# pavlidic/Binary-SpGEMM

Hardware: AMD Instinct MI355X
Metric: output nnz/sec (GNZ/s) (higher is better)
Workload: dtype int32; 1 GPU; R-MAT scale 22, edge factor 16, (a,b,c,d)=(0.30,0.25,0.25,0.20), seed 1, A*A; n=4194304, nnz_a=67108664, products=1336443900, nnz_c=1336366087, parallelism=row-shards x1 cut at equal work, B replicated, priming_steps=0, flow=auto, full=False

## Files before the change

### binary-spgemm_amd/csrc/context.hip

```cpp
#include "internal.hpp"

using namespace bsp;

thread_local char bspgemm_err_text[512] = "";

extern "C" const char *bspgemm_last_error(void) { return g_err; }

extern "C" const char *bspgemm_status_string(bspgemm_status s)
{
    switch (s) {
    case BSPGEMM_OK: return "ok";
    case BSPGEMM_ERR_INVALID: return "invalid argument";
    case BSPGEMM_ERR_ALLOC: return "allocation failed";
    case BSPGEMM_ERR_HIP: return "HIP runtime error";
    case BSPGEMM_ERR_NO_DEVICE: return "no gfx950 device (this library has no CPU fallback)";
    case BSPGEMM_ERR_OVERFLOW: return "result exceeds the int32 drop-in interface";
    case BSPGEMM_ERR_IO: return "file I/O error";
    case BSPGEMM_ERR_FORMAT: return "Matrix Market banner rejected";
    case BSPGEMM_ERR_SIZE: return "Matrix Market size line or entry rejected";
    case BSPGEMM_ERR_COMM: return "RCCL error";
    }
    return "unknown status";
}

// ... 25 lines not shown
        drop();
        hipFree(m->d_col_pad); hipFree(m->d_row_ptr_pad); hipFree(m->d_ext);
        m->d_col_pad = nullptr; m->d_row_ptr_pad = nullptr; m->d_ext = nullptr;
        return st;
    };
    HIPCHK_B(hipMalloc(reinterpret_cast<void **>(&plen), rows * sizeof(int)));
    HIPCHK_B(hipMalloc(reinterpret_cast<void **>(&pp64), (rows + 1) * sizeof(long long)));
    HIPCHK_B(hipMalloc(reinterpret_cast<void **>(&partials), (rows / 2048 + 4) * sizeof(long long)));
    launch_pad_lengths(m->d_row_ptr, m->rows, plen, s);
    launch_scan_counts(plen, m->rows, pp64, partials, nullptr, s);
    long long total = 0;
    HIPCHK_B(hipMemcpyAsync(&total, pp64 + rows, sizeof(long long), hipMemcpyDeviceToHost, s));
    HIPCHK_B(hipStreamSynchronize(s));
    if (total > 0x7fffffffll - 64 || (force < 0 && total > 2 * m->nnz)) { drop(); return BSPGEMM_OK; }
    hipError_t e = hipMalloc(reinterpret_cast<void **>(&m->d_col_pad), ((size_t)total + 64) * sizeof(int));
    if (e == hipSuccess) e = hipMalloc(reinterpret_cast<void **>(&m->d_row_ptr_pad), (rows + 1) * sizeof(int));
    if (e == hipSuccess) e = hipMalloc(reinterpret_cast<void **>(&m->d_ext), rows * sizeof(int2));
    if (e != hipSuccess) {
        (void)hipGetLastError();
        if (force == 1) { snprintf(g_err, sizeof g_err, "padded copy of col_idx: %s", hipGetErrorString(e)); return bail(BSPGEMM_ERR_ALLOC); }
        (void)bail(BSPGEMM_OK);
        return BSPGEMM_OK;
    }
    launch_narrow_row_ptr(pp64, m->d_row_ptr_pad, m->rows + 1, s);
    launch_pad_copy(m->d_row_ptr, m->d_col_idx, m->d_row_ptr_pad, m->rows, m->d_col_pad, m->d_ext, s);
    HIPCHK_B(hipGetLastError());
    HIPCHK_B(hipStreamSynchronize(s));
    drop();
    m->nnz_pad = total;
    m->pad_state = 1;
    return BSPGEMM_OK;
}

bspgemm_status ensure_blk8(const bspgemm_matrix *m)
{
    if (m->blk8_state) return BSPGEMM_OK;
    m->blk8_state = 2;
    const int force = m->ctx->rw_blk;
    if (force == 0 || (force < 0 && m->rows < (1 << 21))) return BSPGEMM_OK;
    const size_t ints = (size_t)3 * (((size_t)m->rows + 7) / 8 + 1);
    HIPCHK(hipMalloc(reinterpret_cast<void **>(&m->d_blk8), (ints + 4) * sizeof(int)));
    unsigned long long *d_clamped = reinterpret_cast<unsigned long long *>(m->d_blk8 + ((ints + 1) & ~(size_t)1));
    HIPCHK(hipMemsetAsync(d_clamped, 0, sizeof(unsigned long long), m->ctx->stream));
    launch_blk8(m->d_row_ptr, m->pad_state == 1 ? m->d_row_ptr_pad : nullptr, m->rows, m->d_blk8, d_clamped, m->ctx->stream);
    HIPCHK(hipGetLastError());
    unsigned long long clamped = 0;
    HIPCHK(hipMemcpyAsync(&clamped, d_clamped, sizeof(clamped), hipMemcpyDeviceToHost, m->ctx->stream));
    HIPCHK(hipStreamSynchronize(m->ctx->stream));
    if (force == 1 || clamped * 8ull <= (unsigned long long)m->nnz) m->blk8_state = 1;
    return BSPGEMM_OK;
}

bspgemm_status use_device(bspgemm_context *ctx)
{
    HIPCHK(hipSetDevice(ctx->device));
    return BSPGEMM_OK;
}

extern "C" int bspgemm_device_count(void)
{
    int ndev = 0;
    if (hipGetDeviceCount(&ndev) != hipSuccess) { (void)hipGetLastError(); return 0; }
    return ndev;
}

extern "C" bspgemm_status bspgemm_create(int device, bspgemm_context **out)
{
    if (!out) return FAIL(BSPGEMM_ERR_INVALID, "ctx is NULL");
    *out = nullptr;
    int ndev = 0;
    if (hipGetDeviceCount(&ndev) != hipSuccess || ndev <= 0)
        return FAIL(BSPGEMM_ERR_NO_DEVICE, "no HIP device visible");
    if (device < 0 || device >= ndev) return FAIL(BSPGEMM_ERR_INVALID, "device index out of range");
    hipDeviceProp_t prop;
    HIPCHK(hipGetDeviceProperties(&prop, device));
    if (strncmp(prop.gcnArchName, "gfx950", 6) != 0) {
        snprintf(g_err, sizeof g_err, "device %d is %s; libbspgemm carries gfx950 code only", device,
                 prop.gcnArchName);
        return BSPGEMM_ERR_NO_DEVICE;
    }
    bspgemm_context *ctx = new (std::nothrow) bspgemm_context();
    if (!ctx) return FAIL(BSPGEMM_ERR_ALLOC, "context");
// ... 105 lines not shown
    HIPCHK_B(hipMalloc(reinterpret_cast<void **>(&m->d_col_idx), ((size_t)nnz + 1) * sizeof(int)));
    HIPCHK_B(hipMemcpyAsync(m->d_row_ptr, row_ptr, ((size_t)rows + 1) * sizeof(int), hipMemcpyHostToDevice, ctx->stream));
    if (nnz > 0)
        HIPCHK_B(hipMemcpyAsync(m->d_col_idx, col_idx + base, (size_t)nnz * sizeof(int), hipMemcpyHostToDevice, ctx->stream));
    launch_rebase_i32(m->d_row_ptr, rows + 1, (int)base, ctx->stream);
    if (bspgemm_status st = ensure_deg8(m)) return bail(st);
    HIPCHK_B(hipStreamSynchronize(ctx->stream));
    *out = m;
    return BSPGEMM_OK;
}

extern "C" bspgemm_status bspgemm_matrix_wrap_device(bspgemm_context *ctx, int rows, int cols, int64_t nnz,
                                                     const int *d_row_ptr, const int *d_col_idx,
                                                     bspgemm_matrix **out)
{
    if (!ctx || !out || !d_row_ptr || rows < 0 || cols < 0 || nnz < 0) return FAIL(BSPGEMM_ERR_INVALID, "matrix_wrap_device");
    bspgemm_matrix *m = new (std::nothrow) bspgemm_matrix{ctx, rows, cols, (long long)nnz,
                                                          const_cast<int *>(d_row_ptr),
                                                          const_cast<int *>(d_col_idx), false};
    if (!m) return FAIL(BSPGEMM_ERR_ALLOC, "matrix");
    *out = m;
    return BSPGEMM_OK;
}

extern "C" void bspgemm_matrix_free(bspgemm_matrix *m)
{
    if (!m) return;
    hipSetDevice(m->ctx->device);
    if (m->owned) {
        hipFree(m->d_row_ptr);
        hipFree(m->d_col_idx);
    }
    hipFree(m->d_deg8);
    hipFree(m->d_blk8);
    hipFree(m->d_col_pad);
    hipFree(m->d_row_ptr_pad);
    hipFree(m->d_ext);
    delete m;
}
extern "C" bspgemm_status bspgemm_matrix_download(bspgemm_context *ctx, const bspgemm_matrix *m, int *row_ptr, int *col_idx)
{
    if (!ctx || !m || m->ctx != ctx) return FAIL(BSPGEMM_ERR_INVALID, "matrix_download");
    if (bspgemm_status st = use_device(ctx)) return st;
    if (row_ptr)
        HIPCHK(hipMemcpyAsync(row_ptr, m->d_row_ptr, ((size_t)m->rows + 1) * sizeof(int), hipMemcpyDeviceToHost, ctx->stream));
    if (col_idx && m->nnz > 0)
        HIPCHK(hipMemcpyAsync(col_idx, m->d_col_idx, (size_t)m->nnz * sizeof(int), hipMemcpyDeviceToHost, ctx->stream));
    HIPCHK(hipStreamSynchronize(ctx->stream));
    return BSPGEMM_OK;
}

extern "C" bspgemm_status bspgemm_matrix_invalidate(bspgemm_matrix *m)
{
    if (!m) return FAIL(BSPGEMM_ERR_INVALID, "matrix is NULL");
    if (bspgemm_status st = use_device(m->ctx)) return st;
    HIPCHK(hipStreamSynchronize(m->ctx->stream));
    hipFree(m->d_deg8);
    hipFree(m->d_blk8);
    hipFree(m->d_col_pad);
    hipFree(m->d_row_ptr_pad);
    hipFree(m->d_ext);
    m->d_deg8 = nullptr;
    m->d_blk8 = nullptr;
    m->blk8_state = 0;
    m->d_col_pad = nullptr;
    m->d_row_ptr_pad = nullptr;
    m->d_ext = nullptr;
    m->pad_state = 0;
    m->nnz_pad = 0;
    return BSPGEMM_OK;
}

extern "C" const char *bspgemm_build_info(void)
{
    return "libbspgemm: HIP kernels for gfx950 only; flows upper-bound (default), exact; small-product path; "
           "timing-only ablation switches: none (BSP_ABLATE=0); tuning constants are compile-time";
}

extern "C" int bspgemm_matrix_rows(const bspgemm_matrix *m) { return m ? m->rows : 0; }
extern "C" int bspgemm_matrix_cols(const bspgemm_matrix *m) { return m ? m->cols : 0; }
extern "C" int64_t bspgemm_matrix_nnz(const bspgemm_matrix *m) { return m ? m->nnz : 0; }

bspgemm_status ensure_rows(bspgemm_context *ctx, size_t rows)
{
    if (rows <= ctx->rows_cap) return BSPGEMM_OK;
    HIPCHK(hipStreamSynchronize(ctx->stream));
    hipFree(ctx->F); hipFree(ctx->Fprefix); hipFree(ctx->partials); hipFree(ctx->cnt); hipFree(ctx->bin_tiles);
    hipFree(ctx->rec); hipFree(ctx->recpre); hipFree(ctx->Fmask); hipFree(ctx->hpartials);
    ctx->F = ctx->Fprefix = ctx->partials = ctx->recpre = ctx->Fmask = ctx->hpartials = nullptr;
    ctx->cnt = ctx->bin_tiles = nullptr;
    ctx->rec = nullptr;
    ctx->rows_cap = 0;
    const size_t cap = rows + rows / 8 + 64;
    const size_t tiles = cap / 2048 + 2;
    HIPCHK(hipMalloc(reinterpret_cast<void **>(&ctx->F), cap * sizeof(long long)));
    HIPCHK(hipMalloc(reinterpret_cast<void **>(&ctx->Fmask), cap * sizeof(long long)));
    HIPCHK(hipMalloc(reinterpret_cast<void **>(&ctx->Fprefix), (cap + 1) * sizeof(long long)));
// ... 223 lines not shown
    case BSPGEMM_OPT_SMALL_PATH:
        if (value < -1 || value > 1) return FAIL(BSPGEMM_ERR_INVALID, "small path: -1, 0 or 1");
        ctx->small = value;
        return BSPGEMM_OK;
    case BSPGEMM_OPT_PADDED_ROWS:
        if (value < -1 || value > 1) return FAIL(BSPGEMM_ERR_INVALID, "padded rows: -1, 0 or 1");
        ctx->pad_rows = value;
        return BSPGEMM_OK;
    }
    return FAIL(BSPGEMM_ERR_INVALID, "unknown option");
}

extern "C" int bspgemm_get_option(const bspgemm_context *ctx, bspgemm_option opt)
{
    if (!ctx) return INT_MIN;
    switch (opt) {
    case BSPGEMM_OPT_CLASS_STREAMS: return ctx->class_streams;
    case BSPGEMM_OPT_BLOCKED_EXTENTS: return ctx->rw_blk;
    case BSPGEMM_OPT_CHECK: return ctx->check ? 1 : 0;
    case BSPGEMM_OPT_SMALL_PATH: return ctx->small;
    case BSPGEMM_OPT_PADDED_ROWS: return ctx->pad_rows;
    }
    return INT_MIN;
}

extern "C" int bspgemm_matrix_uses_padded_rows(const bspgemm_matrix *m)
{
    if (!m || m->pad_state == 0) return -1;
    return m->pad_state == 1 ? 1 : 0;
}

extern "C" int bspgemm_matrix_uses_blocked_table(const bspgemm_matrix *m)
{
    if (!m || m->blk8_state == 0) return -1;
    return m->blk8_state == 1 ? 1 : 0;
}

extern "C" bspgemm_status bspgemm_set_flow(bspgemm_context *ctx, int flow)
{
    if (!ctx || flow < BSPGEMM_FLOW_AUTO || flow > BSPGEMM_FLOW_EXACT) return FAIL(BSPGEMM_ERR_INVALID, "set_flow");
    ctx->flow = flow;
    return BSPGEMM_OK;
}

extern "C" int bspgemm_result_rows(const bspgemm_result *C) { return C ? C->rows : 0; }
extern "C" int64_t bspgemm_result_nnz(const bspgemm_result *C) { return C ? C->nnz : 0; }
extern "C" const int64_t *bspgemm_result_row_ptr_device(const bspgemm_result *C)
{
    return C ? reinterpret_cast<const int64_t *>(C->d_row_ptr) : nullptr;
}
extern "C" const int *bspgemm_result_col_idx_device(const bspgemm_result *C) { return C ? C->d_col_idx : nullptr; }
extern "C" const int *bspgemm_result_values_device(const bspgemm_result *C) { return C ? C->d_values : nullptr; }

extern "C" bspgemm_status bspgemm_result_download(bspgemm_context *ctx, const bspgemm_result *C,
                                                  int64_t *row_ptr, int *col_idx)
{
    if (!ctx || !C) return FAIL(BSPGEMM_ERR_INVALID, "result_download");
    if (bspgemm_status st = use_device(ctx)) return st;
    if (row_ptr)
        HIPCHK(hipMemcpyAsync(row_ptr, C->d_row_ptr, ((size_t)C->rows + 1) * sizeof(long long), hipMemcpyDeviceToHost, ctx->stream));
    if (col_idx && C->nnz > 0)
        HIPCHK(hipMemcpyAsync(col_idx, C->d_col_idx, (size_t)C->nnz * sizeof(int), hipMemcpyDeviceToHost, ctx->stream));
    HIPCHK(hipStreamSynchronize(ctx->stream));
    return BSPGEMM_OK;
}

extern "C" bspgemm_status bspgemm_result_download_values(bspgemm_context *ctx, const bspgemm_result *C, int *values)
{
// ... 34 lines not shown
```

### binary-spgemm_amd/csrc/internal.hpp

```cpp
#pragma once
#include "../../include/bspgemm.h"
#include "kernels.hpp"

#include <hip/hip_runtime.h>

#include <climits>
#include <cstdio>
#include <cstdlib>
#include <cstring>
#include <chrono>
#include <new>

extern thread_local char bspgemm_err_text[512];
#define g_err bspgemm_err_text

static inline bspgemm_status fail(bspgemm_status st, const char *what, const char *file, int line)
{
    snprintf(g_err, sizeof g_err, "%s (%s:%d)", what, file, line);
    return st;
}
#define FAIL(st, what) fail((st), (what), __FILE__, __LINE__)
#define HIPCHK(call)                                                                       \
    do {                                                                                   \
        hipError_t e_ = (call);                                                            \
// ... 71 lines not shown
    int *tmpv = nullptr;
    PrepScalars *d_prep = nullptr;
    bsp::SmallScalars *d_small = nullptr;
    bsp::SmallTiles *d_small_tiles = nullptr;
    unsigned *d_err = nullptr;
    int *chunk_row = nullptr;
    size_t chunk_cap = 0;
    HostScalars *h = nullptr;
    struct CachedBuf { void *p; size_t bytes; };
    CachedBuf cache[8] = {};
    size_t cache_budget = 0;
    int flow = BSPGEMM_FLOW_AUTO;
    bool class_timing = false;
    int class_streams = 2;
    bool check = false;
    int rw_blk = -1;
    int pad_rows = 0;
    int small = -1;
    bool debug_alloc = false;
    bool dropin_timing = false;
};

extern "C" int bspgemm_par_max_plus_one(const int *idx, long long n);
extern "C" void bspgemm_par_prefault(void *p, size_t bytes);
extern "C" long long bspgemm_par_output_bound(const int *Acol, const int *Arow, int r0, int r1, const int *Brow, int brows, long long cap);

struct bspgemm_matrix {
    bspgemm_context *ctx;
    int rows, cols;
    long long nnz;
    int *d_row_ptr, *d_col_idx;
    bool owned;
    mutable unsigned char *d_deg8 = nullptr;
    mutable int *d_blk8 = nullptr;
    mutable int blk8_state = 0;
    mutable int *d_col_pad = nullptr;
    mutable int *d_row_ptr_pad = nullptr;
    mutable int2 *d_ext = nullptr;
    mutable int pad_state = 0;
    mutable long long nnz_pad = 0;
    const int *gather_col() const { return pad_state == 1 ? d_col_pad : d_col_idx; }
    long long gather_nnz() const { return pad_state == 1 ? nnz_pad : nnz; }
};

bspgemm_status ensure_deg8(const bspgemm_matrix *m);
bspgemm_status ensure_blk8(const bspgemm_matrix *m);
bspgemm_status ensure_pad(const bspgemm_matrix *m);

struct bspgemm_result {
    bspgemm_context *ctx;
    int rows;
    long long nnz;
    long long *d_row_ptr;
    int *d_col_idx;
    long long col_cap;
    int *d_values = nullptr;
};

bspgemm_status use_device(bspgemm_context *ctx);

bspgemm_status ensure_rows(bspgemm_context *ctx, size_t rows);
bspgemm_status ensure_ab(bspgemm_context *ctx, size_t pairs);
bspgemm_status ensure_tile_rows(bspgemm_context *ctx, size_t items);
bspgemm_status ensure_tmp(bspgemm_context *ctx, size_t ints);
bspgemm_status ensure_tmpv(bspgemm_context *ctx, size_t ints);
bspgemm_status ensure_chunk_rows(bspgemm_context *ctx, size_t entries);
bool result_cached(const bspgemm_context *ctx, size_t bytes);
hipError_t result_alloc(bspgemm_context *ctx, void **out, size_t bytes);
void result_release(bspgemm_context *ctx, void *p, size_t bytes);
static inline size_t result_bytes_rowptr(int rows) { return ((size_t)rows + 1) * sizeof(long long); }
static inline size_t result_bytes_colidx(long long nnz) { return ((size_t)nnz + 4) * sizeof(int); }

int dropin_fail(const char *fn, bspgemm_status st);
```

### binary-spgemm_amd/csrc/kernels.hpp

```cpp
#pragma once
#include <hip/hip_runtime.h>
#include <stdint.h>
#include <stdlib.h>

namespace bsp {

enum class MaskMode { None, Keep, Drop, Insert, Count };

constexpr int kWaveBins = 16;
constexpr int kNumBins = kWaveBins + 4;
constexpr int kRankBin = kWaveBins + 1;
constexpr int kMidBin = kWaveBins + 2;
constexpr int kDenseBin = kWaveBins + 3;
constexpr int kRankCap = 6144;
int rank_cap_for_cols(long long cols);
constexpr int kMaxBins = 20;
constexpr int kWaveChunks[kWaveBins + 1] = {0, 1, 2, 3, 4, 5, 6, 7, 8, 10, 12, 14, 16, 20, 24, 28, 32};
constexpr int kMaxWaveCap = 64 * kWaveChunks[kWaveBins];
constexpr int kMidCap = 524288;
inline int mid_cap_for_cols(long long cols)
{
    const long long passes = (cols + (1ll << 18) - 1) >> 18;
    if (passes <= 1) return kMidCap;
    const long long c = kMidCap / passes;
    return c < kMaxWaveCap ? kMaxWaveCap : (int)c;
}
constexpr int kRowsPerWave = 16;

constexpr int kWaveTopWords = 256;

inline int levels_for_cols(int64_t cols)
{
    for (int L = 1; L < 5; L++)
        if (cols <= ((int64_t)kWaveTopWords << (5 * L))) return L;
    return 5;
}

constexpr int kWaveTopWordsWide = 512;
inline int wave_levels_for_cols(int64_t cols)
{
    const int L = levels_for_cols(cols);
    if (L == 4 && cols <= ((int64_t)kWaveTopWordsWide << 15)) return 3;
    return L;
}

struct RowRec {
    int row;
    int a0;
    int alen;
    int f;
};

constexpr int kRowWorkTile = 4096;
void launch_row_work(const int *Arow, const int *Acol, const int *Brow, const int *Bblk8, const int *Bpad, const int2 *Bext,
                     int row_begin, int row_end, long long nnz_bound, int *tile_row, long long *F, int2 *ab, hipStream_t s);
void launch_blk8(const int *row_ptr, const int *start_ptr, int n, int *blk, unsigned long long *clamped_nnz, hipStream_t s);
void launch_pad_lengths(const int *row_ptr, int n, int *plen, hipStream_t s);
void launch_pad_copy(const int *row_ptr, const int *col_idx, const int *pad_ptr, int n, int *col_pad, int2 *ext, hipStream_t s);

void launch_deg8(const int *row_ptr, int n, unsigned char *deg8, hipStream_t s);
void launch_row_products(const int *Arow, const int *Acol, const int *Brow, const unsigned char *Bdeg8,
                         int row_begin, int row_end, long long *F, hipStream_t s);

struct PrepScalars {
    long long totalF;
    long long heavy_total;
    long long products;
    int a_lo, a_hi;
    int bin_count[kNumBins];
    unsigned long long max_f;
};
void launch_scan_and_bin(const long long *F, int n, int row_begin, const int *Arow, long long *prefix,
                         long long *partials, int *bin_tiles, int *bin_count, RowRec *rec,
                         long long *recpre, int *cnt, int heavy_cols, long long *hpartials, int mid_cap, int rank_cap, int bound_cols,
                         hipStream_t s, PrepScalars *scal = nullptr, const long long *true_F = nullptr);

constexpr int kCompactGran = 4096;
inline size_t compact_chunk_rows(long long max_out) { return (size_t)((max_out + kCompactGran - 1) / kCompactGran) + 2; }
void launch_scan_counts(const int *cnt, int n, long long *prefix, long long *partials,
                        const long long *base, hipStream_t s, int *chunk_row = nullptr);

constexpr unsigned kErrCapacity = 1u;
constexpr unsigned kErrStaleTable = 2u;
hipError_t launch_wave_rows(int bin, int levels, const int2 *ab, const int *Bcol, int cols,
                            const RowRec *rec, const long long *recpre, const long long *row_ptr, int nrows,
                            int row_begin, int *tmp, int *cnt, unsigned *err, MaskMode mode, const int *Frow, const int *Fcol,
                            hipStream_t s, bool count_only = false);
void launch_check_tables(const int *row_ptr, int rows, const unsigned char *deg8, const int *blk8, const int *pad_ptr, unsigned *err,
                         hipStream_t s);

void launch_place_heavy(const int *tmp, const RowRec *rec, const long long *recpre, int nrows,
                        const long long *row_ptr, int row_begin, int *col_idx, hipStream_t s);

hipError_t launch_dense_rows(int bin, const int2 *ab, const int *Bcol, long long nnzB, int cols,
                             const RowRec *rec, const long long *recpre, int nrows, int row_begin,
                             int *tmp, int *cnt, MaskMode mode, const int *Frow, const int *Fcol, hipStream_t s,
                             int *vals = nullptr);

constexpr int kHeavySortMax = 8192;
void launch_order_heavy(const RowRec *rec, const long long *recpre, int n, RowRec *rec_out, long long *pre_out, hipStream_t s);

bool wave_masked_supported(int cols);
void launch_wave_masked(int bin, const int2 *ab, const int *Bcol, int cols, const int *Frow, const int *Fcol,
                        const RowRec *rec, const long long *recpre, int nrows, int row_begin,
                        int *tmp, int *cnt, int *vals, hipStream_t s);
hipError_t launch_class(int bin, const int2 *ab, const int *Bcol, long long nnzB, int cols, const RowRec *rec,
                        const long long *recpre, int nrows, int row_begin, int *tmp, int *cnt, unsigned *err, MaskMode mode,
                        const int *Frow, const int *Fcol, hipStream_t s, bool count_only = false, int *vals = nullptr);
void launch_mask_lengths(const long long *F, const int *Frow, int row_begin, int n, long long *mlen, hipStream_t s);
void launch_mask_lengths_count(const long long *F, const int *Frow, int row_begin, int n, long long *mlen,
                               unsigned long long *maxF, hipStream_t s);
void launch_insert_lengths(const long long *F, const int *Drow, int row_begin, int n, long long *size, hipStream_t s);

void launch_compact(const int *tmp, const long long *Fprefix, const long long *row_ptr,
                    int row_lo, int row_hi, long long max_out, int *col_idx, hipStream_t s, const int *chunk_row = nullptr);

constexpr int kSmallMaxProducts = 65536;
constexpr int kSmallMaxRow = 2048;
constexpr int kSmallMaxRows = 1 << 17;
constexpr int kSmallMaxNnzA = 32768;
struct SmallScalars {
// ... 35 lines not shown
```

### binary-spgemm_amd/csrc/multiply.hip

```cpp
#include "internal.hpp"

using namespace bsp;

static bspgemm_status check_operands(bspgemm_context *ctx, const bspgemm_matrix *A, const bspgemm_matrix *B,
                                     int row_begin, int row_end)
{
    if (!ctx || !A || !B) return FAIL(BSPGEMM_ERR_INVALID, "NULL operand");
    if (A->ctx != ctx || B->ctx != ctx) return FAIL(BSPGEMM_ERR_INVALID, "operand belongs to another context");
    if (row_begin < 0 || row_end < row_begin || row_end > A->rows) return FAIL(BSPGEMM_ERR_INVALID, "row range");
    if (B->rows < A->cols) return FAIL(BSPGEMM_ERR_INVALID, "B has fewer rows than A has columns");
    return BSPGEMM_OK;
}


static void class_order(const int *bin_count, long long total_products, int *order, int *lane)
{
    int light[kWaveBins];
    for (int k = 0; k < kWaveBins; k++) light[k] = k + 1;
    const long long heavy_lower_bound = ((long long)bin_count[kRankBin] + bin_count[kMidBin] + bin_count[kDenseBin]) * kMaxWaveCap;
    if (heavy_lower_bound * 8 < total_products) {
        long long key[kNumBins] = {};
        for (int b = 1; b <= kWaveBins; b++) key[b] = (long long)bin_count[b] * kWaveChunks[b];
        for (int a = 1; a < kWaveBins; a++)
            for (int c = a; c > 0 && key[light[c]] > key[light[c - 1]]; c--) {
// ... 60 lines not shown
    return st;
}

static hipError_t alloc_col_idx(bspgemm_context *ctx, bspgemm_result *C, long long cap)
{
    if (hipError_t e = result_alloc(ctx, reinterpret_cast<void **>(&C->d_col_idx), result_bytes_colidx(cap))) return e;
    C->col_cap = cap;
    return hipSuccess;
}
static long long col_cap_for(long long bound, long long nnz_c) { return (bound - nnz_c <= nnz_c / 50 + 4096) ? bound : nnz_c; }

static bspgemm_status start_flow(bspgemm_context *ctx, const bspgemm_matrix *A, const bspgemm_matrix *B,
                                 const bspgemm_matrix *Fm, int row_begin, int row_end, int flow, bspgemm_result **out,
                                 bspgemm_result **Cp)
{
    if (!out) return FAIL(BSPGEMM_ERR_INVALID, "result pointer is NULL");
    *out = nullptr;
    if (bspgemm_status st = check_operands(ctx, A, B, row_begin, row_end)) return st;
    if (Fm && (Fm->ctx != ctx || Fm->rows < row_end)) return FAIL(BSPGEMM_ERR_INVALID, "mask has fewer rows than A / wrong context");
    if (bspgemm_status st = use_device(ctx)) return st;
    const int R = row_end - row_begin;
    hipStream_t s = ctx->stream;
    if (bspgemm_status st = ensure_rows(ctx, (size_t)R + 1)) return st;
    if (bspgemm_status st = ensure_ab(ctx, (size_t)A->nnz + 1)) return st;
    if (bspgemm_status st = ensure_tile_rows(ctx, (size_t)A->nnz + (size_t)R)) return st;

    bspgemm_result *C = new (std::nothrow) bspgemm_result{ctx, R, 0, nullptr, nullptr, 0};
    if (!C) return FAIL(BSPGEMM_ERR_ALLOC, "result");
    auto bail = [&](bspgemm_status st) { return drop_result(C, st); };
    bspgemm_context::StatSlot &slot = open_slot(ctx, flow, false);
    HIPCHK_B(hipEventRecord(slot.ev[0], s));
    HIPCHK_B(result_alloc(ctx, reinterpret_cast<void **>(&C->d_row_ptr), result_bytes_rowptr(R)));
    if (bspgemm_status st = ensure_pad(B)) return bail(st);
    if (bspgemm_status st = ensure_blk8(B)) return bail(st);
    if (ctx->check) {
        HIPCHK_B(hipMemsetAsync(ctx->d_err, 0, sizeof(unsigned), s));
        launch_check_tables(B->d_row_ptr, B->rows, B->d_deg8, B->blk8_state == 1 ? B->d_blk8 : nullptr,
                            B->pad_state == 1 ? B->d_row_ptr_pad : nullptr, ctx->d_err, s);
    }
    slot.prepass_kernel = B->blk8_state == 1 ? 1 : 0;
    slot.padded = B->pad_state == 1;
    launch_row_work(A->d_row_ptr, A->d_col_idx, B->d_row_ptr, B->blk8_state == 1 ? B->d_blk8 : nullptr,
                    B->pad_state == 1 ? B->d_row_ptr_pad : nullptr, B->pad_state == 1 ? B->d_ext : nullptr, row_begin, row_end,
                    A->nnz, ctx->tile_row, ctx->F, ctx->ab, s);
    *Cp = C;
    return BSPGEMM_OK;
}

template <class Launch>
static bspgemm_status class_phase(bspgemm_context *ctx, int phase, long long products, int *cls_n, bool heavy_on_third,
                                  Launch launch)
{
    const int *bin_count = ctx->h->bin_count;
    hipStream_t lanes[3] = {ctx->stream, ctx->stream_b, ctx->stream_c};
    const int nlanes = ctx->class_streams;
    hipEvent_t *tile = ctx->ev_tile[phase];
    hipEvent_t (*ev_cls)[2] = ctx->slots[ctx->slot_head].ev_cls[phase];
    size_t bin_start[kNumBins + 1] = {0, 0};
    for (int b = 1; b < kNumBins; b++) bin_start[b + 1] = bin_start[b] + (size_t)bin_count[b];
    int order[kNumBins], lane_of[kNumBins];
    class_order(bin_count, products, order, lane_of);

    HIPCHK(hipEventRecord(tile[0], lanes[0]));
    for (int l = 1; l < 3; l++)
        if (l < nlanes || (l == 2 && heavy_on_third)) HIPCHK(hipStreamWaitEvent(lanes[l], tile[0], 0));
    for (int pos = 1; pos < kNumBins; pos++) {
        const int b = order[pos];
        const int n = bin_count[b];
        cls_n[b] = n;
        if (n <= 0) continue;
        hipStream_t sx = heavy_on_third && b > kWaveBins ? lanes[2] : lanes[lane_of[pos] % nlanes];
        if (ctx->class_timing) HIPCHK(hipEventRecord(ev_cls[b][0], sx));
        HIPCHK(launch(b, n, ctx->rec + bin_start[b], ctx->recpre + bin_start[b], sx));
        if (ctx->class_timing) HIPCHK(hipEventRecord(ev_cls[b][1], sx));
    }
// ... 486 lines not shown
```

### binary-spgemm_amd/csrc/prepass.hip

```cpp
#include "kernels.hpp"
#include "wave.hpp"

namespace bsp {

struct __attribute__((packed, aligned(4))) Int2U { int x, y; };

constexpr int kLongRow = 256;
constexpr int kRowWorkUnroll = 4;
template <typename Sweep>
__device__ __forceinline__ long long rows_of_a_wave(int a0, int a1, int sub, Sweep &&sweep)
{
    const int lane = threadIdx.x & 63;
    long long long_sum = 0;
#pragma unroll
    for (int q = 0; q < 8; q++) {
        const int qa0 = __builtin_amdgcn_readlane(a0, q * 8), qa1 = __builtin_amdgcn_readlane(a1, q * 8);
        if (qa1 - qa0 > kLongRow) {
            long long t = sweep((long long)qa0 + lane, (long long)qa1, 64);
#pragma unroll
            for (int d = 1; d < 64; d <<= 1) t += __shfl_xor(t, d, 64);
            if (lane == q * 8) long_sum = t;
        }
    }
    const bool is_long = a1 - a0 > kLongRow;
// ... 18 lines not shown
    const int sub = (int)(gid & 7);
    int a0 = 0, a1 = 0;
    if (r < nrows) { a0 = Arow[row_begin + r]; a1 = Arow[row_begin + r + 1]; }
    constexpr int U = kRowWorkUnroll;
    auto sweep = [&](long long first, long long end, int stride) {
        long long sum = 0;
        for (long long jj = first; jj < end; jj += (long long)stride * U) {
            int j[U];
#pragma unroll
            for (int u = 0; u < U; u++) j[u] = (jj + stride * u < end) ? Acol[jj + stride * u] : -1;
            Int2U pr[U];
#pragma unroll
            for (int u = 0; u < U; u++) {
                pr[u].x = pr[u].y = 0;
                if (j[u] >= 0) {
                    if (PAD) { const int2 e = Bext[j[u]]; pr[u].x = e.x; pr[u].y = e.x + e.y; }
                    else pr[u] = *reinterpret_cast<const Int2U *>(Brow + j[u]);
                }
            }
#pragma unroll
            for (int u = 0; u < U; u++)
                if (j[u] >= 0) {
                    const int len = pr[u].y - pr[u].x;
                    ab[jj + stride * u] = make_int2(pr[u].x, len);
                    sum += (long long)len;
                }
        }
        return sum;
    };
    const long long sum = rows_of_a_wave(a0, a1, sub, sweep);
    if (r < nrows && sub == 0) F[r] = sum;
}

struct __attribute__((packed, aligned(4))) Blk8 { int base; unsigned lo, hi; };

__global__ __launch_bounds__(256) void k_blk8(const int *__restrict__ row_ptr, const int *__restrict__ start_ptr, int n,
                                              int *__restrict__ blk, unsigned long long *__restrict__ clamped_nnz)
{
    const int b = blockIdx.x * blockDim.x + threadIdx.x;
    if (b * 8 >= n) return;
    const int r0 = b * 8;
    unsigned lo = 0u, hi = 0u;
    long long clamped = 0;
    int prev = row_ptr[r0];
    const int base = start_ptr[r0];
#pragma unroll
    for (int k = 0; k < 8; k++) {
        int d = 0;
        if (r0 + k < n) {
            const int nx = row_ptr[r0 + k + 1];
            d = nx - prev;
            prev = nx;
        }
        const unsigned byte = (unsigned)(d < 255 ? d : 255);
        if (d >= 255) clamped += d;
        if (k < 4) lo |= byte << (8 * k); else hi |= byte << (8 * (k - 4));
    }
    if (clamped > 0) atomicAdd(clamped_nnz, (unsigned long long)clamped);
    blk[3 * b] = base;
    blk[3 * b + 1] = (int)lo;
    blk[3 * b + 2] = (int)hi;
}
void launch_blk8(const int *row_ptr, const int *start_ptr, int n, int *blk, unsigned long long *clamped_nnz, hipStream_t s)
{
    if (n <= 0) return;
    const int nb = (n + 7) / 8;
    hipLaunchKernelGGL(k_blk8, dim3((nb + 255) / 256), dim3(256), 0, s, row_ptr, start_ptr ? start_ptr : row_ptr, n, blk, clamped_nnz);
}

template <bool PAD>
__device__ __forceinline__ void blk8_extent(const Blk8 &w, int j, int &start, int &len, bool &sat)
{
    const int k = j & 7;
    const u64 d = ((u64)w.hi << 32) | (u64)w.lo;
    const u64 below = d & ((1ull << (8 * k)) - 1ull);
    const u64 upto = (k == 7) ? d : (d & ((1ull << (8 * k + 8)) - 1ull));
    const u64 v = ~upto;
    sat = ((v - 0x0101010101010101ull) & ~v & 0x8080808080808080ull) != 0ull;
    if (PAD) {
        const u64 m0f = 0x0f0f0f0f0f0f0f0full, m01 = 0x0101010101010101ull;
        const u64 units = ((below >> 4) & m0f) + ((((below & m0f) + m0f) >> 4) & m01);
        start = w.base + 16 * ((int)__builtin_amdgcn_sad_u8((unsigned)units, 0u, 0u)
                               + (int)__builtin_amdgcn_sad_u8((unsigned)(units >> 32), 0u, 0u));
    } else {
        start = w.base + (int)__builtin_amdgcn_sad_u8((unsigned)below, 0u, 0u)
                + (int)__builtin_amdgcn_sad_u8((unsigned)(below >> 32), 0u, 0u);
    }
    len = (int)((d >> (8 * k)) & 255ull);
}

constexpr int kFlatTile = kRowWorkTile;
constexpr int kFlatK = kFlatTile / 256;

__global__ __launch_bounds__(256) void k_tile_rows(const int *__restrict__ Arow, int row_begin, int nrows,
                                                   int *__restrict__ tile_row, long long *__restrict__ F)
{
    const int r = blockIdx.x * blockDim.x + threadIdx.x;
    if (r >= nrows) return;
    const long long lo = Arow[row_begin];
    const long long m0 = Arow[row_begin + r] - lo + r, m1 = Arow[row_begin + r + 1] - lo + r;
    for (long long t = (m0 + kFlatTile - 1) / kFlatTile; t * kFlatTile <= m1; t++) tile_row[t] = r;
    if (m0 / kFlatTile != m1 / kFlatTile) F[r] = 0;
}

template <bool PAD>
__global__ __launch_bounds__(256) void k_row_work_flat(const int *__restrict__ Arow,
                                                       const int *__restrict__ Acol,
                                                       const int *__restrict__ Brow,
                                                       const int *__restrict__ Bblk,
                                                       const int *__restrict__ Bpad,
                                                       int row_begin, int nrows,
                                                       const int *__restrict__ tile_row,
                                                       long long *__restrict__ F,
                                                       int2 *__restrict__ ab)
{
    constexpr int K = kFlatK, NB = kFlatTile, RV = kFlatK + 1;
    constexpr int LSTRIDE = K + 4;
    __shared__ __attribute__((aligned(16))) long long P[NB + NB / 16 + 1];
    __shared__ long long wsum[4];
    static_assert(256 * LSTRIDE * sizeof(int) <= sizeof(P), "staged lengths do not fit the prefix array");
    int *L = reinterpret_cast<int *>(P);
    auto pidx = [](int q) { return q + (q >> 4); };

    const int tid = threadIdx.x;
    const int *rp = Arow + row_begin;
    const long long lo = rp[0], nnz = rp[nrows] - lo, total = nnz + nrows;
    const long long d0 = (long long)blockIdx.x * NB;
    if (d0 >= total) return;
    const bool last = d0 + NB >= total;
    const long long d1 = last ? total : d0 + NB;
    const int rb = tile_row[blockIdx.x];
    const int rl = last ? nrows - 1 : tile_row[blockIdx.x + 1];
    const long long j0 = d0 - rb, j1 = last ? nnz : d1 - rl;
    const int n = (int)(j1 - j0);
    const long long g0 = lo + j0;
    int fa0 = 0, fa1 = 0;
    if (rb + tid <= rl) { fa0 = rp[rb + tid]; fa1 = rp[rb + tid + 1]; }

    int j[K];
#pragma unroll
    for (int k = 0; k < K; k++) j[k] = tid + 256 * k < n ? Acol[g0 + tid + 256 * k] : -1;
    Blk8 w[K];
#pragma unroll
    for (int k = 0; k < K; k++) {
        w[k].base = 0; w[k].lo = w[k].hi = 0u;
        if (j[k] >= 0) w[k] = *reinterpret_cast<const Blk8 *>(Bblk + 3 * (j[k] >> 3));
    }
    int start[K], len[K];
    bool sat[K];
#pragma unroll
    for (int k = 0; k < K; k++) {
        blk8_extent<PAD>(w[k], j[k], start[k], len[k], sat[k]);
        sat[k] = sat[k] && j[k] >= 0;
    }
    Int2U pr[K];
    int ps[K];
#pragma unroll
    for (int k = 0; k < K; k++) {
        pr[k].x = pr[k].y = 0;
        ps[k] = 0;
        if (sat[k]) {
            pr[k] = *reinterpret_cast<const Int2U *>(Brow + j[k]);
            if (PAD) ps[k] = Bpad[j[k]];
        }
    }
#pragma unroll
    for (int k = 0; k < K; k++) {
        const int p = tid + 256 * k;
        if (sat[k]) { start[k] = PAD ? ps[k] : pr[k].x; len[k] = pr[k].y - pr[k].x; }
        if (j[k] < 0) len[k] = 0;
        else ab[g0 + p] = make_int2(start[k], len[k]);
        L[p + 4 * (p / K)] = len[k];
    }
    __syncthreads();

    int mine[K];
#pragma unroll
    for (int i = 0; i < K; i += 4) {
        const int4 v = *reinterpret_cast<const int4 *>(L + LSTRIDE * tid + i);
        mine[i] = v.x; mine[i + 1] = v.y; mine[i + 2] = v.z; mine[i + 3] = v.w;
    }
    long long tot = 0;
#pragma unroll
    for (int i = 0; i < K; i++) tot += mine[i];
    const long long inc = wave_incl_scan64(tot);
    const int lane = tid & 63, wv = tid >> 6;
    if (lane == 63) wsum[wv] = inc;
    __syncthreads();
    long long off = inc - tot;
    for (int k = 0; k < wv; k++) off += wsum[k];
#pragma unroll
    for (int i = 0; i < K; i++) {
        off += mine[i];
        P[pidx(K * tid + i + 1)] = off;
    }
    if (tid == 0) P[0] = 0;
    int ra0[RV], ra1[RV];
    ra0[0] = fa0;
    ra1[0] = fa1;
#pragma unroll
    for (int i = 1; i < RV; i++)
        if (rb + tid + 256 * i <= rl) { ra0[i] = rp[rb + tid + 256 * i]; ra1[i] = rp[rb + tid + 256 * i + 1]; }
    __syncthreads();

#pragma unroll
    for (int i = 0; i < RV; i++) {
        const int r = rb + tid + 256 * i;
        if (r > rl) break;
        const long long a0 = ra0[i] - lo, a1 = ra1[i] - lo;
        const long long s = a0 > j0 ? a0 : j0, e = a1 < j1 ? a1 : j1;
        const long long v = e > s ? P[pidx((int)(e - j0))] - P[pidx((int)(s - j0))] : 0;
        if (a0 + r >= d0 && a1 + r < d1) F[r] = v;
        else if (v != 0) atomicAdd(reinterpret_cast<unsigned long long *>(F + r), (unsigned long long)v);
    }
}

void launch_row_work(const int *Arow, const int *Acol, const int *Brow, const int *Bblk8, const int *Bpad, const int2 *Bext,
                     int row_begin, int row_end, long long nnz_bound, int *tile_row, long long *F, int2 *ab, hipStream_t s)
{
    const int nrows = row_end - row_begin;
    if (nrows <= 0) return;
    if (Bblk8) {
        hipLaunchKernelGGL(k_tile_rows, dim3((nrows + 255) / 256), dim3(256), 0, s, Arow, row_begin, nrows, tile_row, F);
        const int tiles = (int)((nnz_bound + nrows + kFlatTile - 1) / kFlatTile);
        if (Bpad)
            hipLaunchKernelGGL(k_row_work_flat<true>, dim3(tiles), dim3(256), 0, s, Arow, Acol, Brow, Bblk8, Bpad, row_begin, nrows,
                               tile_row, F, ab);
        else
            hipLaunchKernelGGL(k_row_work_flat<false>, dim3(tiles), dim3(256), 0, s, Arow, Acol, Brow, Bblk8, nullptr, row_begin,
                               nrows, tile_row, F, ab);
        return;
    }
    const long long threads = (long long)nrows * 8;
    const int grid = (int)((threads + 255) / 256);
    if (Bext)
        hipLaunchKernelGGL(k_row_work<true>, dim3(grid), dim3(256), 0, s, Arow, Acol, Brow, Bext, row_begin, nrows, F, ab);
    else
        hipLaunchKernelGGL(k_row_work<false>, dim3(grid), dim3(256), 0, s, Arow, Acol, Brow, nullptr, row_begin, nrows, F, ab);
}

__global__ __launch_bounds__(256) void k_pad_lengths(const int *__restrict__ row_ptr, int n, int *__restrict__ plen)
{
    const int i = blockIdx.x * blockDim.x + threadIdx.x;
    if (i < n) plen[i] = ((row_ptr[i + 1] - row_ptr[i]) + 15) & ~15;
}
void launch_pad_lengths(const int *row_ptr, int n, int *plen, hipStream_t s)
{
    if (n <= 0) return;
    hipLaunchKernelGGL(k_pad_lengths, dim3((n + 255) / 256), dim3(256), 0, s, row_ptr, n, plen);
}
__global__ __launch_bounds__(256) void k_pad_copy(const int *__restrict__ row_ptr, const int *__restrict__ col_idx,
                                                  const int *__restrict__ pad_ptr, int n, int *__restrict__ col_pad,
                                                  int2 *__restrict__ ext)
{
    const long long gid = (long long)blockIdx.x * blockDim.x + threadIdx.x;
    const int r = (int)(gid >> 4), sub = (int)(gid & 15);
    if (r >= n) return;
    const int s0 = row_ptr[r], len = row_ptr[r + 1] - s0, d0 = pad_ptr[r];
    const int plen = (len + 15) & ~15;
    for (int t = sub; t < plen; t += 16) col_pad[d0 + t] = col_idx[s0 + (t < len ? t : len - 1)];
    if (sub == 0 && ext) ext[r] = make_int2(d0, len);
}
// ... 31 lines not shown
    constexpr int U = 4;
    auto sweep = [&](long long first, long long end, int stride) {
        long long sum = 0;
        for (long long jj = first; jj < end; jj += (long long)stride * U) {
            int j[U];
#pragma unroll
            for (int u = 0; u < U; u++) j[u] = (jj + stride * u < end) ? Acol[jj + stride * u] : -1;
            int d[U];
#pragma unroll
            for (int u = 0; u < U; u++) d[u] = j[u] >= 0 ? (int)Bdeg8[j[u]] : 0;
#pragma unroll
            for (int u = 0; u < U; u++) {
                if (d[u] == 255) d[u] = Brow[j[u] + 1] - Brow[j[u]];
                sum += (long long)d[u];
            }
        }
        return sum;
    };
    const long long sum = rows_of_a_wave(a0, a1, sub, sweep);
    if (r < nrows && sub == 0) F[r] = sum;
}

__global__ __launch_bounds__(256) void k_check_tables(const int *__restrict__ row_ptr, int n,
                                                      const unsigned char *__restrict__ deg8, const int *__restrict__ blk,
                                                      const int *__restrict__ pad_ptr, unsigned *__restrict__ err)
{
    const int i = blockIdx.x * blockDim.x + threadIdx.x;
    if (i >= n) return;
    const int d = row_ptr[i + 1] - row_ptr[i];
    const unsigned want = (unsigned)(d < 255 ? d : 255);
    bool bad = d < 0;
    if (deg8) bad = bad || deg8[i] != want;
    if (blk) {
        const int b = i >> 3, k = i & 7;
        const unsigned w = (unsigned)blk[3 * b + 1 + (k >> 2)];
        bad = bad || ((w >> (8 * (k & 3))) & 255u) != want || (k == 0 && blk[3 * b] != (pad_ptr ? pad_ptr[i] : row_ptr[i]));
    }
    if (pad_ptr) bad = bad || pad_ptr[i + 1] - pad_ptr[i] != ((d + 15) & ~15);
    if (bad) atomicOr(err, kErrStaleTable);
}
void launch_check_tables(const int *row_ptr, int rows, const unsigned char *deg8, const int *blk8, const int *pad_ptr, unsigned *err,
                         hipStream_t s)
{
    if (rows <= 0 || (!deg8 && !blk8 && !pad_ptr)) return;
    hipLaunchKernelGGL(k_check_tables, dim3((rows + 255) / 256), dim3(256), 0, s, row_ptr, rows, deg8, blk8, pad_ptr, err);
}

void launch_row_products(const int *Arow, const int *Acol, const int *Brow, const unsigned char *Bdeg8,
                         int row_begin, int row_end, long long *F, hipStream_t s)
{
    const int nrows = row_end - row_begin;
    if (nrows <= 0) return;
    const long long threads = (long long)nrows * 8;
    hipLaunchKernelGGL(k_row_products, dim3((int)((threads + 255) / 256)), dim3(256), 0, s, Arow, Acol, Brow, Bdeg8,
                       row_begin, nrows, F);
}

__global__ __launch_bounds__(256) void k_insert_lengths(const long long *__restrict__ F, const int *__restrict__ Drow, int row_begin,
                                                        int n, long long *__restrict__ size)
{
    const int i = blockIdx.x * blockDim.x + threadIdx.x;
    if (i < n) size[i] = F[i] + (long long)(Drow[row_begin + i + 1] - Drow[row_begin + i]);
}

void launch_insert_lengths(const long long *F, const int *Drow, int row_begin, int n, long long *size, hipStream_t s)
{
    if (n <= 0) return;
    hipLaunchKernelGGL(k_insert_lengths, dim3((n + 255) / 256), dim3(256), 0, s, F, Drow, row_begin, n, size);
}

constexpr int kScanThreads = 256;
constexpr int kScanItems = 8;
constexpr int kScanTile = kScanThreads * kScanItems;

__device__ __forceinline__ int bin_of(long long F, int mid_cap, int rank_cap)
{
    if (F <= 0) return 0;
    if (F > kMaxWaveCap) return F <= rank_cap ? kRankBin : (F > mid_cap ? kDenseBin : kMidBin);
// ... 303 lines not shown
```

Measured before the change: 228.4 GNZ/s.

## Replace 8-row byte-packed degree table with 16-row 6-bit packed int4 table

The blocked extent table for B now packs 16 rows per 16-byte int4: one base offset plus 16 six-bit clamped degrees, instead of 8 rows with 8-bit degrees in 12 bytes. The table shrinks per row and each lookup becomes one aligned 16-byte load, cutting the gather traffic from random column indices. The 6-bit clamp at 63 sends many more R-MAT rows to the saturated fallback that reads row_ptr directly, and the enable threshold is relaxed to allow more clamped nnz. Loads of A columns and stores of the (start,len) pairs also become nontemporal.

```diff
diff --git a/binary-spgemm_amd/csrc/context.hip b/binary-spgemm_amd/csrc/context.hip
--- a/binary-spgemm_amd/csrc/context.hip
+++ b/binary-spgemm_amd/csrc/context.hip
@@ -81,22 +81,22 @@
     return BSPGEMM_OK;
 }
 
-bspgemm_status ensure_blk8(const bspgemm_matrix *m)
-{
-    if (m->blk8_state) return BSPGEMM_OK;
-    m->blk8_state = 2;
+bspgemm_status ensure_blk16(const bspgemm_matrix *m)
+{
+    if (m->blk16_state) return BSPGEMM_OK;
+    m->blk16_state = 2;
     const int force = m->ctx->rw_blk;
     if (force == 0 || (force < 0 && m->rows < (1 << 21))) return BSPGEMM_OK;
-    const size_t ints = (size_t)3 * (((size_t)m->rows + 7) / 8 + 1);
-    HIPCHK(hipMalloc(reinterpret_cast<void **>(&m->d_blk8), (ints + 4) * sizeof(int)));
-    unsigned long long *d_clamped = reinterpret_cast<unsigned long long *>(m->d_blk8 + ((ints + 1) & ~(size_t)1));
+    const size_t ints = (size_t)4 * (((size_t)m->rows + 15) / 16 + 1);
+    HIPCHK(hipMalloc(reinterpret_cast<void **>(&m->d_blk16), (ints + 4) * sizeof(int)));
+    unsigned long long *d_clamped = reinterpret_cast<unsigned long long *>(m->d_blk16 + ints);
     HIPCHK(hipMemsetAsync(d_clamped, 0, sizeof(unsigned long long), m->ctx->stream));
-    launch_blk8(m->d_row_ptr, m->pad_state == 1 ? m->d_row_ptr_pad : nullptr, m->rows, m->d_blk8, d_clamped, m->ctx->stream);
+    launch_blk16(m->d_row_ptr, m->pad_state == 1 ? m->d_row_ptr_pad : nullptr, m->rows, m->d_blk16, d_clamped, m->ctx->stream);
     HIPCHK(hipGetLastError());
     unsigned long long clamped = 0;
     HIPCHK(hipMemcpyAsync(&clamped, d_clamped, sizeof(clamped), hipMemcpyDeviceToHost, m->ctx->stream));
     HIPCHK(hipStreamSynchronize(m->ctx->stream));
-    if (force == 1 || clamped * 8ull <= (unsigned long long)m->nnz) m->blk8_state = 1;
+    if (force == 1 || clamped * 4ull <= (unsigned long long)m->nnz) m->blk16_state = 1;
     return BSPGEMM_OK;
 }
 
@@ -268,7 +268,7 @@
         hipFree(m->d_col_idx);
     }
     hipFree(m->d_deg8);
-    hipFree(m->d_blk8);
+    hipFree(m->d_blk16);
     hipFree(m->d_col_pad);
     hipFree(m->d_row_ptr_pad);
     hipFree(m->d_ext);
@@ -292,13 +292,13 @@
     if (bspgemm_status st = use_device(m->ctx)) return st;
     HIPCHK(hipStreamSynchronize(m->ctx->stream));
     hipFree(m->d_deg8);
-    hipFree(m->d_blk8);
+    hipFree(m->d_blk16);
     hipFree(m->d_col_pad);
     hipFree(m->d_row_ptr_pad);
     hipFree(m->d_ext);
     m->d_deg8 = nullptr;
-    m->d_blk8 = nullptr;
-    m->blk8_state = 0;
+    m->d_blk16 = nullptr;
+    m->blk16_state = 0;
     m->d_col_pad = nullptr;
     m->d_row_ptr_pad = nullptr;
     m->d_ext = nullptr;
@@ -588,8 +588,8 @@
 
 extern "C" int bspgemm_matrix_uses_blocked_table(const bspgemm_matrix *m)
 {
-    if (!m || m->blk8_state == 0) return -1;
-    return m->blk8_state == 1 ? 1 : 0;
+    if (!m || m->blk16_state == 0) return -1;
+    return m->blk16_state == 1 ? 1 : 0;
 }
 
 extern "C" bspgemm_status bspgemm_set_flow(bspgemm_context *ctx, int flow)
diff --git a/binary-spgemm_amd/csrc/internal.hpp b/binary-spgemm_amd/csrc/internal.hpp
--- a/binary-spgemm_amd/csrc/internal.hpp
+++ b/binary-spgemm_amd/csrc/internal.hpp
@@ -127,8 +127,8 @@
     int *d_row_ptr, *d_col_idx;
     bool owned;
     mutable unsigned char *d_deg8 = nullptr;
-    mutable int *d_blk8 = nullptr;
-    mutable int blk8_state = 0;
+    mutable int *d_blk16 = nullptr;
+    mutable int blk16_state = 0;
     mutable int *d_col_pad = nullptr;
     mutable int *d_row_ptr_pad = nullptr;
     mutable int2 *d_ext = nullptr;
@@ -139,7 +139,7 @@
 };
 
 bspgemm_status ensure_deg8(const bspgemm_matrix *m);
-bspgemm_status ensure_blk8(const bspgemm_matrix *m);
+bspgemm_status ensure_blk16(const bspgemm_matrix *m);
 bspgemm_status ensure_pad(const bspgemm_matrix *m);
 
 struct bspgemm_result {
diff --git a/binary-spgemm_amd/csrc/kernels.hpp b/binary-spgemm_amd/csrc/kernels.hpp
--- a/binary-spgemm_amd/csrc/kernels.hpp
+++ b/binary-spgemm_amd/csrc/kernels.hpp
@@ -52,9 +52,9 @@
 };
 
 constexpr int kRowWorkTile = 4096;
-void launch_row_work(const int *Arow, const int *Acol, const int *Brow, const int *Bblk8, const int *Bpad, const int2 *Bext,
+void launch_row_work(const int *Arow, const int *Acol, const int *Brow, const int *Bblk16, const int *Bpad, const int2 *Bext,
                      int row_begin, int row_end, long long nnz_bound, int *tile_row, long long *F, int2 *ab, hipStream_t s);
-void launch_blk8(const int *row_ptr, const int *start_ptr, int n, int *blk, unsigned long long *clamped_nnz, hipStream_t s);
+void launch_blk16(const int *row_ptr, const int *start_ptr, int n, int *blk, unsigned long long *clamped_nnz, hipStream_t s);
 void launch_pad_lengths(const int *row_ptr, int n, int *plen, hipStream_t s);
 void launch_pad_copy(const int *row_ptr, const int *col_idx, const int *pad_ptr, int n, int *col_pad, int2 *ext, hipStream_t s);
 
@@ -86,7 +86,7 @@
                             const RowRec *rec, const long long *recpre, const long long *row_ptr, int nrows,
                             int row_begin, int *tmp, int *cnt, unsigned *err, MaskMode mode, const int *Frow, const int *Fcol,
                             hipStream_t s, bool count_only = false);
-void launch_check_tables(const int *row_ptr, int rows, const unsigned char *deg8, const int *blk8, const int *pad_ptr, unsigned *err,
+void launch_check_tables(const int *row_ptr, int rows, const unsigned char *deg8, const int *blk16, const int *pad_ptr, unsigned *err,
                          hipStream_t s);
 
 void launch_place_heavy(const int *tmp, const RowRec *rec, const long long *recpre, int nrows,
diff --git a/binary-spgemm_amd/csrc/multiply.hip b/binary-spgemm_amd/csrc/multiply.hip
--- a/binary-spgemm_amd/csrc/multiply.hip
+++ b/binary-spgemm_amd/csrc/multiply.hip
@@ -116,15 +116,15 @@
     HIPCHK_B(hipEventRecord(slot.ev[0], s));
     HIPCHK_B(result_alloc(ctx, reinterpret_cast<void **>(&C->d_row_ptr), result_bytes_rowptr(R)));
     if (bspgemm_status st = ensure_pad(B)) return bail(st);
-    if (bspgemm_status st = ensure_blk8(B)) return bail(st);
+    if (bspgemm_status st = ensure_blk16(B)) return bail(st);
     if (ctx->check) {
         HIPCHK_B(hipMemsetAsync(ctx->d_err, 0, sizeof(unsigned), s));
-        launch_check_tables(B->d_row_ptr, B->rows, B->d_deg8, B->blk8_state == 1 ? B->d_blk8 : nullptr,
+        launch_check_tables(B->d_row_ptr, B->rows, B->d_deg8, B->blk16_state == 1 ? B->d_blk16 : nullptr,
                             B->pad_state == 1 ? B->d_row_ptr_pad : nullptr, ctx->d_err, s);
     }
-    slot.prepass_kernel = B->blk8_state == 1 ? 1 : 0;
+    slot.prepass_kernel = B->blk16_state == 1 ? 1 : 0;
     slot.padded = B->pad_state == 1;
-    launch_row_work(A->d_row_ptr, A->d_col_idx, B->d_row_ptr, B->blk8_state == 1 ? B->d_blk8 : nullptr,
+    launch_row_work(A->d_row_ptr, A->d_col_idx, B->d_row_ptr, B->blk16_state == 1 ? B->d_blk16 : nullptr,
                     B->pad_state == 1 ? B->d_row_ptr_pad : nullptr, B->pad_state == 1 ? B->d_ext : nullptr, row_begin, row_end,
                     A->nnz, ctx->tile_row, ctx->F, ctx->ab, s);
     *Cp = C;
diff --git a/binary-spgemm_amd/csrc/prepass.hip b/binary-spgemm_amd/csrc/prepass.hip
--- a/binary-spgemm_amd/csrc/prepass.hip
+++ b/binary-spgemm_amd/csrc/prepass.hip
@@ -74,61 +74,72 @@
     if (r < nrows && sub == 0) F[r] = sum;
 }
 
-struct __attribute__((packed, aligned(4))) Blk8 { int base; unsigned lo, hi; };
-
-__global__ __launch_bounds__(256) void k_blk8(const int *__restrict__ row_ptr, const int *__restrict__ start_ptr, int n,
-                                              int *__restrict__ blk, unsigned long long *__restrict__ clamped_nnz)
-{
-    const int b = blockIdx.x * blockDim.x + threadIdx.x;
-    if (b * 8 >= n) return;
-    const int r0 = b * 8;
-    unsigned lo = 0u, hi = 0u;
+constexpr int kBlkClamp = 63;
+
+__device__ __forceinline__ unsigned blk16_field(int d) { return (unsigned)(d < kBlkClamp ? d : kBlkClamp); }
+
+__global__ __launch_bounds__(256) void k_blk16(const int *__restrict__ row_ptr, const int *__restrict__ start_ptr, int n,
+                                               int4 *__restrict__ blk, unsigned long long *__restrict__ clamped_nnz)
+{
+    const int g = blockIdx.x * blockDim.x + threadIdx.x;
+    if ((long long)g * 16 >= n) return;
+    const int r0 = g * 16;
+    unsigned w[3] = {0u, 0u, 0u};
     long long clamped = 0;
     int prev = row_ptr[r0];
     const int base = start_ptr[r0];
 #pragma unroll
-    for (int k = 0; k < 8; k++) {
+    for (int k = 0; k < 16; k++) {
         int d = 0;
         if (r0 + k < n) {
             const int nx = row_ptr[r0 + k + 1];
             d = nx - prev;
             prev = nx;
         }
-        const unsigned byte = (unsigned)(d < 255 ? d : 255);
-        if (d >= 255) clamped += d;
-        if (k < 4) lo |= byte << (8 * k); else hi |= byte << (8 * (k - 4));
+        const unsigned f = blk16_field(d);
+        if (d >= kBlkClamp) clamped += d;
+        if (k < 15) w[k / 5] |= f << (6 * (k % 5));
+        else { w[0] |= (f & 3u) << 30; w[1] |= ((f >> 2) & 3u) << 30; w[2] |= (f >> 4) << 30; }
     }
     if (clamped > 0) atomicAdd(clamped_nnz, (unsigned long long)clamped);
-    blk[3 * b] = base;
-    blk[3 * b + 1] = (int)lo;
-    blk[3 * b + 2] = (int)hi;
-}
-void launch_blk8(const int *row_ptr, const int *start_ptr, int n, int *blk, unsigned long long *clamped_nnz, hipStream_t s)
+    blk[g] = make_int4(base, (int)w[0], (int)w[1], (int)w[2]);
+}
+void launch_blk16(const int *row_ptr, const int *start_ptr, int n, int *blk, unsigned long long *clamped_nnz, hipStream_t s)
 {
     if (n <= 0) return;
-    const int nb = (n + 7) / 8;
-    hipLaunchKernelGGL(k_blk8, dim3((nb + 255) / 256), dim3(256), 0, s, row_ptr, start_ptr ? start_ptr : row_ptr, n, blk, clamped_nnz);
+    const int ng = (n + 15) / 16;
+    hipLaunchKernelGGL(k_blk16, dim3((ng + 255) / 256), dim3(256), 0, s, row_ptr, start_ptr ? start_ptr : row_ptr, n,
+                       reinterpret_cast<int4 *>(blk), clamped_nnz);
+}
+
+__device__ __forceinline__ unsigned blk16_last(unsigned w0, unsigned w1, unsigned w2)
+{
+    return (w0 >> 30) | ((w1 >> 30) << 2) | ((w2 >> 30) << 4);
 }
 
 template <bool PAD>
-__device__ __forceinline__ void blk8_extent(const Blk8 &w, int j, int &start, int &len, bool &sat)
-{
-    const int k = j & 7;
-    const u64 d = ((u64)w.hi << 32) | (u64)w.lo;
-    const u64 below = d & ((1ull << (8 * k)) - 1ull);
-    const u64 upto = (k == 7) ? d : (d & ((1ull << (8 * k + 8)) - 1ull));
-    const u64 v = ~upto;
-    sat = ((v - 0x0101010101010101ull) & ~v & 0x8080808080808080ull) != 0ull;
+__device__ __forceinline__ void blk16_extent(const int4 &g, int j, int &start, int &len, bool &sat)
+{
+    const unsigned w0 = (unsigned)g.y, w1 = (unsigned)g.z, w2 = (unsigned)g.w;
+    const int k = j & 15, t = 6 * k;
+    const int b0 = min(t, 30), b1 = min(max(t - 30, 0), 30), b2 = min(max(t - 60, 0), 30);
+    const unsigned x0 = w0 & ((1u << b0) - 1u), x1 = w1 & ((1u << b1) - 1u), x2 = w2 & ((1u << b2) - 1u);
     if (PAD) {
-        const u64 m0f = 0x0f0f0f0f0f0f0f0full, m01 = 0x0101010101010101ull;
-        const u64 units = ((below >> 4) & m0f) + ((((below & m0f) + m0f) >> 4) & m01);
-        start = w.base + 16 * ((int)__builtin_amdgcn_sad_u8((unsigned)units, 0u, 0u)
-                               + (int)__builtin_amdgcn_sad_u8((unsigned)(units >> 32), 0u, 0u));
+        auto units = [](unsigned x) {
+            return ((x >> 4) & 0x030c30c3u) + ((((x & 0x0f3cf3cfu) + 0x0f3cf3cfu) >> 4) & 0x01041041u);
+        };
+        const unsigned u = units(x0) + units(x1) + units(x2);
+        start = g.x + 16 * (int)(((u * 0x01041041u) >> 24) & 63u);
     } else {
-        start = w.base + (int)__builtin_amdgcn_sad_u8((unsigned)below, 0u, 0u)
-                + (int)__builtin_amdgcn_sad_u8((unsigned)(below >> 32), 0u, 0u);
-    }
-    len = (int)((d >> (8 * k)) & 255ull);
+        const unsigned me = 0x3f03f03fu, mo = 0x00fc0fc0u;
+        const unsigned e = (x0 & me) + (x1 & me) + (x2 & me), o = (x0 & mo) + (x1 & mo) + (x2 & mo);
+        start = g.x + (int)((e & 0xfffu) + ((e >> 12) & 0xfffu) + (e >> 24) + ((o >> 6) & 0xfffu) + (o >> 18));
+    }
+    const unsigned wk = k < 5 ? w0 : (k < 10 ? w1 : w2);
+    const int sh = t - (k < 5 ? 0 : (k < 10 ? 30 : 60));
+    len = k == 15 ? (int)blk16_last(w0, w1, w2) : (int)((wk >> sh) & 63u);
+    auto full = [](unsigned x) { return (~x - 0x01041041u) & x & 0x20820820u; };
+    sat = ((full(x0) | full(x1) | full(x2)) != 0u) || len == kBlkClamp;
 }
 
 constexpr int kFlatTile = kRowWorkTile;
@@ -181,18 +192,18 @@
 
     int j[K];
 #pragma unroll
-    for (int k = 0; k < K; k++) j[k] = tid + 256 * k < n ? Acol[g0 + tid + 256 * k] : -1;
-    Blk8 w[K];
+    for (int k = 0; k < K; k++) j[k] = tid + 256 * k < n ? __builtin_nontemporal_load(Acol + g0 + tid + 256 * k) : -1;
+    int4 w[K];
 #pragma unroll
     for (int k = 0; k < K; k++) {
-        w[k].base = 0; w[k].lo = w[k].hi = 0u;
-        if (j[k] >= 0) w[k] = *reinterpret_cast<const Blk8 *>(Bblk + 3 * (j[k] >> 3));
+        w[k] = make_int4(0, 0, 0, 0);
+        if (j[k] >= 0) w[k] = reinterpret_cast<const int4 *>(Bblk)[j[k] >> 4];
     }
     int start[K], len[K];
     bool sat[K];
 #pragma unroll
     for (int k = 0; k < K; k++) {
-        blk8_extent<PAD>(w[k], j[k], start[k], len[k], sat[k]);
+        blk16_extent<PAD>(w[k], j[k], start[k], len[k], sat[k]);
         sat[k] = sat[k] && j[k] >= 0;
     }
     Int2U pr[K];
@@ -211,7 +222,9 @@
         const int p = tid + 256 * k;
         if (sat[k]) { start[k] = PAD ? ps[k] : pr[k].x; len[k] = pr[k].y - pr[k].x; }
         if (j[k] < 0) len[k] = 0;
-        else ab[g0 + p] = make_int2(start[k], len[k]);
+        else
+            __builtin_nontemporal_store((long long)(((u64)(unsigned)len[k] << 32) | (u64)(unsigned)start[k]),
+                                        reinterpret_cast<long long *>(ab + g0 + p));
         L[p + 4 * (p / K)] = len[k];
     }
     __syncthreads();
@@ -257,19 +270,19 @@
     }
 }
 
-void launch_row_work(const int *Arow, const int *Acol, const int *Brow, const int *Bblk8, const int *Bpad, const int2 *Bext,
+void launch_row_work(const int *Arow, const int *Acol, const int *Brow, const int *Bblk16, const int *Bpad, const int2 *Bext,
                      int row_begin, int row_end, long long nnz_bound, int *tile_row, long long *F, int2 *ab, hipStream_t s)
 {
     const int nrows = row_end - row_begin;
     if (nrows <= 0) return;
-    if (Bblk8) {
+    if (Bblk16) {
         hipLaunchKernelGGL(k_tile_rows, dim3((nrows + 255) / 256), dim3(256), 0, s, Arow, row_begin, nrows, tile_row, F);
         const int tiles = (int)((nnz_bound + nrows + kFlatTile - 1) / kFlatTile);
         if (Bpad)
-            hipLaunchKernelGGL(k_row_work_flat<true>, dim3(tiles), dim3(256), 0, s, Arow, Acol, Brow, Bblk8, Bpad, row_begin, nrows,
+            hipLaunchKernelGGL(k_row_work_flat<true>, dim3(tiles), dim3(256), 0, s, Arow, Acol, Brow, Bblk16, Bpad, row_begin, nrows,
                                tile_row, F, ab);
         else
-            hipLaunchKernelGGL(k_row_work_flat<false>, dim3(tiles), dim3(256), 0, s, Arow, Acol, Brow, Bblk8, nullptr, row_begin,
+            hipLaunchKernelGGL(k_row_work_flat<false>, dim3(tiles), dim3(256), 0, s, Arow, Acol, Brow, Bblk16, nullptr, row_begin,
                                nrows, tile_row, F, ab);
         return;
     }
@@ -367,18 +380,20 @@
     bool bad = d < 0;
     if (deg8) bad = bad || deg8[i] != want;
     if (blk) {
-        const int b = i >> 3, k = i & 7;
-        const unsigned w = (unsigned)blk[3 * b + 1 + (k >> 2)];
-        bad = bad || ((w >> (8 * (k & 3))) & 255u) != want || (k == 0 && blk[3 * b] != (pad_ptr ? pad_ptr[i] : row_ptr[i]));
+        const int4 g = reinterpret_cast<const int4 *>(blk)[i >> 4];
+        const int k = i & 15;
+        const unsigned w = (unsigned)(k < 5 ? g.y : (k < 10 ? g.z : g.w));
+        const unsigned f = k == 15 ? blk16_last((unsigned)g.y, (unsigned)g.z, (unsigned)g.w) : (w >> (6 * (k % 5))) & 63u;
+        bad = bad || f != blk16_field(d) || (k == 0 && g.x != (pad_ptr ? pad_ptr[i] : row_ptr[i]));
     }
     if (pad_ptr) bad = bad || pad_ptr[i + 1] - pad_ptr[i] != ((d + 15) & ~15);
     if (bad) atomicOr(err, kErrStaleTable);
 }
-void launch_check_tables(const int *row_ptr, int rows, const unsigned char *deg8, const int *blk8, const int *pad_ptr, unsigned *err,
+void launch_check_tables(const int *row_ptr, int rows, const unsigned char *deg8, const int *blk16, const int *pad_ptr, unsigned *err,
                          hipStream_t s)
 {
-    if (rows <= 0 || (!deg8 && !blk8 && !pad_ptr)) return;
-    hipLaunchKernelGGL(k_check_tables, dim3((rows + 255) / 256), dim3(256), 0, s, row_ptr, rows, deg8, blk8, pad_ptr, err);
+    if (rows <= 0 || (!deg8 && !blk16 && !pad_ptr)) return;
+    hipLaunchKernelGGL(k_check_tables, dim3((rows + 255) / 256), dim3(256), 0, s, row_ptr, rows, deg8, blk16, pad_ptr, err);
 }
 
 void launch_row_products(const int *Arow, const int *Acol, const int *Brow, const unsigned char *Bdeg8,
```

New measurement: 235.7 GNZ/s (median of 6 runs). 3.2% higher.
